# avik-pal/LocalRegNeuralDE.jl

Measured on NVIDIA B200. Metric: mnist_ode_train_samples_per_s, higher is better.
Workload: dtype tf32x3

## Files before the change

localregneuralde.jl_b200/csrc/lrnde_adjoint.cu:

```cuda
#include "lrnde_adjoint.h"

#include <stdio.h>
#include <stdlib.h>
#include <string.h>

#include <algorithm>

#include "lrnde_fused_dev.cuh"

enum {
  LA_ALPHA = 0,
  LA_S1 = 2,
  LA_DEL = 8,
  LA_CC = 13,
  LA_HH = 18,
  LA_EPS = 23,
  LA_DBT = 29,
  LA_HBB = 30,
  LA_HBT = 31,
  LA_NARR = 32
};

#ifdef LRNDE_UMMA_TRACE
__device__ long long g_adj_trace[1024];
// ... 158 lines not shown
        }
        bulk_commit();
        bulk_wait0();
      }
      __syncwarp();
    }
  } else if (warp == 1) {
    constexpr uint32_t idesc = make_idesc(128, kNT / 2);
    mbar_wait(&a_ready, 0);
    tc_fence_after();
    const uint32_t mz_hi = tmem_base, mz_lo = tmem_base + (uint32_t)(8 * p.KS);
    const uint32_t mt_hi = tmem_base + (uint32_t)(16 * p.KS), mt_lo = tmem_base + (uint32_t)(24 * p.KS);
    for (int st = 0; st < nst; ++st) {
      const uint32_t ph = (uint32_t)(st & 1);
      for (int cg = 0; cg < 2; ++cg) {
        mbar_wait(&bfull[cg], ph);
        tc_fence_after();
        if (elect_one_sync()) {
          if (cg == 0 && !SINGLE) ATRACE(7, st);
          issue_group(c_acc + (uint32_t)(cg * 32), mz_hi, mz_lo, smem_u32(tC[cg]), p.nfull, p.ntail, p.passes, idesc);
          mma_commit(&pdone[cg]);
          if (cg == 0 && !SINGLE) ATRACE(8, st);
        }
        __syncwarp();
      }
      if (!SINGLE) {
        for (int cg = 0; cg < 2; ++cg) {
          mbar_wait(&pread[cg], ph);
          tc_fence_after();
          if (elect_one_sync()) {
            issue_group(c_acc + (uint32_t)(cg * 32), mt_hi, mt_lo, smem_u32(tE[cg]), p.nfull, p.ntail, p.passes, idesc);
            mma_commit(&xdone[cg]);
          }
          __syncwarp();
        }
      }
    }
  } else {
    const int q = warp & 3, sub = (warp - 2) >> 2;
    const int cg = sub >> 1;
    const int hrow = q * 32 + lane;
    const uint32_t tlane = tmem_base + ((uint32_t)(q * 32) << 16);
    const int rbase = (sub & 1) * 16;
    const int nb = n0 + cg * 32 + rbase;
    const bool rowv = hrow < p.H;
    const bool rowc = hrow < p.Kaug;
    {
#pragma unroll
      for (int j = 0; j < 4; ++j) {
        const int ks = sub + 4 * j;
        if (ks < p.KS) {
          float a1[8], a2[8], hi[8], lo[8];
#pragma unroll
          for (int e = 0; e < 8; ++e) {
            const int k = ks * 8 + e;
            a1[e] = __ldg(p.Mz + hrow * 128 + k);
            a2[e] = (rowv && k < p.H) ? __ldg(p.Mz + k * 128 + hrow) : 0.0f;
          }
#pragma unroll
          for (int e = 0; e < 8; ++e) {
            if (p.passes == 3) { hi[e] = tf32_rna(a1[e]); lo[e] = tf32_rna(a1[e] - hi[e]); }
            else { hi[e] = a1[e]; lo[e] = 0.0f; }
          }
          tmem_st8(tlane + (uint32_t)(ks * 8), hi);
          tmem_st8(tlane + (uint32_t)(8 * p.KS + ks * 8), lo);
#pragma unroll
          for (int e = 0; e < 8; ++e) {
            if (p.passes == 3) { hi[e] = tf32_rna(a2[e]); lo[e] = tf32_rna(a2[e] - hi[e]); }
            else { hi[e] = a2[e]; lo[e] = 0.0f; }
          }
          tmem_st8(tlane + (uint32_t)(16 * p.KS + ks * 8), hi);
          tmem_st8(tlane + (uint32_t)(24 * p.KS + ks * 8), lo);
        }
      }
    }
    tmem_st_wait();
    tc_fence_before();
    __syncwarp();
    if (lane == 0) mbar_arrive(&a_ready);
    if (tr) ATRACE(0, 1);

    const bool in_full = hrow < p.nfull * 32;
    const bool in_img = hrow < p.KS * 8;
    uint32_t oA, oS, oLo, osw;
    if (in_full) {
      oS = 128u; oLo = 4096u; osw = (uint32_t)(lane >> 2);
      oA = (uint32_t)(q * 8192 + (lane & 3) * 4) + (uint32_t)rbase * oS;
    } else {
      const int kt = hrow - p.nfull * 32, t = kt >> 3, kk = kt & 7;
      oS = 32u; oLo = 1024u; osw = (uint32_t)((kk >> 2) & 1);
      oA = (uint32_t)(p.nfull * 8192 + t * 2048 + (kk & 3) * 4) + (uint32_t)rbase * oS;
    }
    const uint32_t rnd = (p.passes == 3) ? 0x1000u : 0u, msk = (p.passes == 3) ? 0xFFFFE000u : 0xFFFFFFFFu;
    auto tile_put16 = [&](uint8_t* tile, const float (&val)[16]) {
      if (!in_img) return;
#pragma unroll
      for (int i = 0; i < 16; ++i) {
        const uint32_t m = in_full ? (uint32_t)(i & 7) : (uint32_t)((i >> 2) & 1);
        const uint32_t o = oA + (uint32_t)i * oS + ((osw ^ m) << 4);
        const float hi = __uint_as_float((__float_as_uint(val[i]) + rnd) & msk);
        const float lo = __uint_as_float((__float_as_uint(val[i] - hi) + rnd) & msk);
        *reinterpret_cast<float*>(tile + o) = hi;
        *reinterpret_cast<float*>(tile + o + oLo) = lo;
      }
    };
    const float w1t = (p.td && rowv && p.w1t) ? p.w1t[hrow] : 0.0f;
    const float b1 = rowv ? p.b1[hrow] : 0.0f;
    const int slot = s_slot, next = s_next;
    const float dt = sd[0].scale;
    const float* alpha_n = SINGLE ? p.alpha_in : arr(LA_ALPHA + slot);
    const size_t e0 = (size_t)nb * LR_ZROW + hrow;
    uint8_t* const tCc = tC[cg];
    uint8_t* const tEc = tE[cg];
    const float* tape_row = reinterpret_cast<const float*>(tbuf) + (cg * 32 + rbase) * LR_ZROW + hrow;

    float c[16], ep[16], dprev[16];
#pragma unroll
    for (int i = 0; i < 16; ++i) { c[i] = 0.0f; ep[i] = 0.0f; dprev[i] = 0.0f; }
    if (!SINGLE && rowv) {
      const float* d1 = arr(LA_S1 + 3 * slot + 0) + e0;
#pragma unroll
      for (int i = 0; i < 16; ++i) dprev[i] = __ldcg(d1 + (size_t)i * LR_ZROW);
    }
    float v[16], ss[16];
    for (int jj = -1; jj < nst; ++jj) {
      const LinComb& yd = SINGLE ? sy[0] : sy[jj < 0 ? 1 : jj + 1];
      const float tau = yd.t;
      const bool last = (!SINGLE && jj == 5);
      float* dst_del = SINGLE ? arr(LA_S1 + 3 * slot + 0) : (last ? arr(LA_S1 + 3 * next + 0) : arr(LA_DEL + max(jj, 0)));
      float* dst_hh = SINGLE ? arr(LA_S1 + 3 * slot + 1) : (last ? arr(LA_S1 + 3 * next + 1) : arr(LA_HH + max(jj, 0)));
      float* dst_cc = SINGLE ? arr(LA_S1 + 3 * slot + 2) : (last ? arr(LA_S1 + 3 * next + 2) : arr(LA_CC + max(jj, 0)));
      if (jj >= 0) {
        if (tr) ATRACE(1, jj);
        const float cextra = (hrow == p.Kaug) ? tau : ((hrow == p.Kaug + 1) ? 1.0f : 0.0f);
#pragma unroll
        for (int i = 0; i < 16; ++i) dst_cc[e0 + (size_t)i * LR_ZROW] = rowc ? c[i] : cextra;
        tile_put16(tCc, c);
        if (!SINGLE) {
          const float cl = sd[jj].coef[jj];
          float* dst_eps = arr(LA_EPS + jj) + e0;
#pragma unroll
          for (int i = 0; i < 16; ++i) { v[i] = fmaf(cl, dprev[i], ep[i]); dst_eps[(size_t)i * LR_ZROW] = v[i]; }
          tile_put16(tEc, v);
        }
        tc_fence_before();
        fence_proxy_async();
        __syncwarp();
        if (lane == 0) mbar_arrive(&bfull[cg]);
        if (tr) ATRACE(2, jj);
      }
      if (jj + 1 < nst) {
        const LinComb& yn = SINGLE ? sy[0] : sy[jj + 2];
#pragma unroll
        for (int i = 0; i < 16; ++i) c[i] = 0.0f;
        for (int s = 0; s < 8; ++s) {
          const int it = (jj + 1) * 8 + s;
          const int b = it % kTapeBufs;
          mbar_wait(&tfull[b], (uint32_t)((it / kTapeBufs) & 1));
          if (rowc) {
            const float* tb = tape_row + (size_t)b * (kTapeBufBytes / 4);
            const float cf = (s < 7) ? yn.coef[s] : 1.0f, sc = (s < 7) ? 1.0f : yn.scale;
#pragma unroll
            for (int i = 0; i < 16; ++i) c[i] = fmaf(cf, tb[i * LR_ZROW], sc * c[i]);
          }
          __syncwarp();
          if (lane == 0) mbar_arrive(&tempty[b]);
        }
        if (!SINGLE && jj >= 0) {
#pragma unroll
          for (int i = 0; i < 16; ++i) ep[i] = sd[jj + 1].coef[jj] * dprev[i];
          if (rowv) {
            for (int s = 0; s < jj; ++s) {
              const float* src = ((s == 0) ? arr(LA_S1 + 3 * slot + 0) : arr(LA_DEL + s - 1)) + e0;
              const float cf = sd[jj + 1].coef[s];
#pragma unroll
              for (int i = 0; i < 16; ++i) ep[i] = fmaf(cf, __ldcg(src + (size_t)i * LR_ZROW), ep[i]);
            }
          }
        }
      }
      if (jj >= 0) {
        if (tr) ATRACE(3, jj);
#pragma unroll
        for (int i = 0; i < 16; ++i) ss[i] = rowv ? __ldcg(p.Zx + e0 + (size_t)i * LR_ZROW) : 0.0f;
        mbar_wait(&pdone[cg], (uint32_t)(jj & 1));
        if (tr) ATRACE(4, jj);
// ... 236 lines not shown
            if (pvec && row + 3 < o.prows) r = __ldcg(reinterpret_cast<const float4*>(pp));
            else {
              if (row + 0 < o.prows) r.x = __ldcg(pp + 0);
              if (row + 1 < o.prows) r.y = __ldcg(pp + 1);
              if (row + 2 < o.prows) r.z = __ldcg(pp + 2);
              if (row + 3 < o.prows) r.w = __ldcg(pp + 3);
            }
          } else if (g < 4) {
            r = __ldcg(reinterpret_cast<const float4*>(o.Q0 + (size_t)b * LR_ZROW + c4 * 4));
          } else if (o.Q1) {
            r = __ldcg(reinterpret_cast<const float4*>(o.Q1 + (size_t)b * LR_ZROW + c4 * 4));
          }
        }
        dst[g] = r;
      }
    };
    if (niter > 0) load_iter(0, v[0]);
    if (niter > 1) load_iter(1, v[1]);
    for (int it0 = 0; it0 < niter; it0 += 2) {
#pragma unroll
      for (int dd = 0; dd < 2; ++dd) {
        const int it = it0 + dd;
        if (it < niter) {
          const int s = it % NS, ph = (it / NS) & 1;
          uint8_t* stage = smem + (size_t)s * kPaStageBytes;
          const Ops o = ops_of(it);
          mbar_wait(&empty_bar[s], (uint32_t)(ph ^ 1));
#pragma unroll
          for (int g = 0; g < 6; ++g) {
            const int li = tid + (g & 1) * PT;
            const int bl = li >> 5, c4 = li & 31;
            const int grp = c4 >> 3, c32 = (c4 & 7) >> 1, half = c4 & 1, k4 = bl >> 2, r = bl & 3;
            const uint32_t off = (uint32_t)((k4 * 4 + grp) * 512 + r * 128 + ((c32 ^ r) << 5) + half * 16);
            float4 xv = (g >= 4 && !o.Q1) ? v[dd][g - 2] : v[dd][g];
            const float sc = (g < 2) ? 1.0f : ((g < 4) ? o.s0 : o.s1);
            xv.x *= sc; xv.y *= sc; xv.z *= sc; xv.w *= sc;
            float4 hi, lo;
            if (q.passes == 3) {
              hi = make_float4(tf32_rna(xv.x), tf32_rna(xv.y), tf32_rna(xv.z), tf32_rna(xv.w));
              lo = make_float4(tf32_rna(xv.x - hi.x), tf32_rna(xv.y - hi.y), tf32_rna(xv.z - hi.z), tf32_rna(xv.w - hi.w));
            } else { hi = xv; lo = make_float4(0.f, 0.f, 0.f, 0.f); }
            uint8_t* img = stage + (g >> 1) * 32768;
            *reinterpret_cast<float4*>(img + off) = hi;
            *reinterpret_cast<float4*>(img + 16384 + off) = lo;
          }
          if (it + 2 < niter) load_iter(it + 2, v[dd]);
          fence_proxy_async();
          __syncwarp();
          if (lane == 0) mbar_arrive(&full_bar[s]);
        }
      }
    }
    mbar_wait(&done_bar, 0);
    tc_fence_after();
    const int quarter = (warp & 3) * 32;
    const int wgroup = (warp - 2) >> 2;
    const int mrow = quarter + lane;
    const int nacc = (job == 0) ? 4 : 2;
    float* out;
    if (job == 0) out = q.partP + (size_t)split * 4 * 16384;
    else out = (job == 1 ? q.partX : q.partL) + ((size_t)split * q.ntile + tile) * 2 * 16384;
    for (int a = 0; a < nacc; ++a) {
      for (int cb = wgroup; cb < 8; cb += kEpiWarps / 4) {
        float r[16];
        tmem_ld16(tmem_base + ((uint32_t)quarter << 16) + (uint32_t)(a * 128 + cb * 16), r);
        float4* o4 = reinterpret_cast<float4*>(out + (size_t)a * 16384 + (size_t)mrow * 128 + cb * 16);
        if (niter == 0) {
#pragma unroll
          for (int j = 0; j < 16; ++j) r[j] = 0.0f;
        }
#pragma unroll
        for (int j = 0; j < 4; ++j) o4[j] = make_float4(r[4 * j], r[4 * j + 1], r[4 * j + 2], r[4 * j + 3]);
      }
    }
    tc_fence_before();
  }
  __syncthreads();
  if (warp == 1) {
    tc_fence_after();
    asm volatile("tcgen05.dealloc.cta_group::1.sync.aligned.b32 %0, %1;" ::"r"(tmem_base), "r"(512u) : "memory");
  }
}

struct AReduceP {
  SolveDev* S;
  const float* partP; const float* partX; const float* partL;
  float* RP; float* RX; float* RL;
  int nP, nD, ntile;
};
__global__ void __launch_bounds__(256) adj_reduce_kernel(AReduceP p) {
  if (p.S->done) return;
  const size_t nP4 = 4 * 4096, nX4 = (size_t)p.ntile * 2 * 4096;
  for (size_t i = blockIdx.x * (size_t)blockDim.x + threadIdx.x; i < nP4 + 2 * nX4; i += (size_t)gridDim.x * blockDim.x) {
    float4 s = make_float4(0.f, 0.f, 0.f, 0.f);
    if (i < nP4) {
      const float4* src = reinterpret_cast<const float4*>(p.partP) + i;
#pragma unroll 8
      for (int k = 0; k < p.nP; ++k) {
        const float4 v = __ldcg(src + (size_t)k * nP4);
        s.x += v.x; s.y += v.y; s.z += v.z; s.w += v.w;
      }
      reinterpret_cast<float4*>(p.RP)[i] = s;
    } else {
      const bool isx = (i - nP4) < nX4;
      const size_t j = isx ? (i - nP4) : (i - nP4 - nX4);
      const float4* src = reinterpret_cast<const float4*>(isx ? p.partX : p.partL) + j;
      for (int k = 0; k < p.nD; ++k) {
        const float4 v = __ldcg(src + (size_t)k * nX4);
        s.x += v.x; s.y += v.y; s.z += v.z; s.w += v.w;
      }
      const size_t tile = j / (2 * 4096), rem = j % (2 * 4096), vv = rem / 4096, mn = rem % 4096;
      float4* dst = reinterpret_cast<float4*>(isx ? p.RX : p.RL);
      dst[(vv * p.ntile + tile) * 4096 + mn] = s;
    }
  }
}

struct AMuP {
  SolveDev* S;
  const float* RP; const float* RX; const float* RL;
  const float* W2a;
  const float* W1T;
  int D, H, td, Kaug, ntile;
  long w1_off, w2_off;
  long nparams;
};
__global__ void __launch_bounds__(512) adj_mu_kernel(AMuP p) {
  SolveDev* S = p.S;
  if (S->done) return;
  const int slot = S->slot, next = (S->slot + 1) % S->cap;
  const float* mu_n = lr_slot_u(S, slot) + S->lam_len;
  float* mu_new = lr_slot_u(S, next) + S->lam_len;
  const float dt = S->err.scale, abstol = S->abstol, reltol = S->reltol;
  const int H = p.H, D = p.D, Kaug = p.Kaug;
  const long n1 = (long)H * (D + p.td + 1), n2 = (long)D * Kaug;
  const size_t RXs = (size_t)p.ntile * 128 * 128;
  const bool multi = S->reduce_mu && S->nranks > 1;
  const int par = (int)(S->mseq & 1ull);
  float* st0 = multi ? lr_mbox_stage(S->mbox[S->rank], par, 0) : nullptr;
  float* st1 = multi ? lr_mbox_stage(S->mbox[S->rank], par, 1) : nullptr;
  double acc = 0.0;
  for (long i = blockIdx.x * (long)blockDim.x + threadIdx.x; i < n1 + n2; i += (long)gridDim.x * blockDim.x) {
    float g0, g1;
    long pidx;
    if (i < n1) {
      const int d = (int)(i / H), r = (int)(i % H);
      pidx = p.w1_off + i;
      if (d < D) {
        float a0 = p.RX[(size_t)d * 128 + r], a1 = p.RX[RXs + (size_t)d * 128 + r];
        const float* w = p.W2a + d;
        const float* P0 = p.RP + r;
        const float* P1 = p.RP + 16384 + r;
#pragma unroll 8
        for (int k = 0; k < Kaug; ++k) {
          const float wv = __ldg(w + (size_t)k * D);
          a0 = fmaf(P0[k * 128], wv, a0);
          a1 = fmaf(P1[k * 128], wv, a1);
        }
        g0 = a0; g1 = a1;
      } else {
        const int krow = (p.td && d == D) ? Kaug : Kaug + 1;
        g0 = p.RP[(size_t)krow * 128 + r];
        g1 = p.RP[16384 + (size_t)krow * 128 + r];
      }
    } else {
      const long i2 = i - n1;
      const int k = (int)(i2 / D), d = (int)(i2 % D);
      pidx = p.w2_off + i2;
      float a0 = 0.0f, a1 = 0.0f;
      const float* P0 = p.RP + 2 * 16384 + (size_t)k * 128;
      const float* P1 = p.RP + 3 * 16384 + (size_t)k * 128;
      const float* w = p.W1T + d;
#pragma unroll 8
      for (int r = 0; r < H; ++r) {
        const float wv = __ldg(w + (size_t)r * D);
        a0 = fmaf(P0[r], wv, a0);
        a1 = fmaf(P1[r], wv, a1);
      }
      g0 = fmaf(-dt, a0, p.RL[(size_t)d * 128 + k]);
      g1 = fmaf(-dt, a1, p.RL[RXs + (size_t)d * 128 + k]);
    }
    if (multi) {
      st0[pidx] = g0;
      st1[pidx] = g1;
      continue;
    }
    const float mn = mu_n[pidx];
    const float mv = fmaf(-dt, g0, mn);
    mu_new[pidx] = mv;
    const float ut = -dt * g1;
    const float r = ut / (abstol + fmaxf(fabsf(mn), fabsf(mv)) * reltol);
    acc += (double)(r * r);
  }
  if (multi) {
    __threadfence_system();
    __syncthreads();
    if (threadIdx.x == 0) {
      const unsigned int prev = atomicAdd(S->mucounter, 1u);
      if (prev == gridDim.x - 1) {
        *S->mucounter = 0;
        __threadfence_system();
        for (int r = 0; r < S->nranks; ++r) {
          volatile unsigned long long* f = &S->mbox[r]->mflag[par][S->rank];
          *f = S->mseq + 1;
        }
      }
    }
    return;
  }
  __shared__ double sh[16];
  for (int o = 16; o > 0; o >>= 1) acc += __shfl_down_sync(0xffffffffu, acc, o);
  if ((threadIdx.x & 31) == 0) sh[threadIdx.x >> 5] = acc;
  __syncthreads();
  if (threadIdx.x == 0) {
    double s = 0.0;
    for (int w = 0; w < (int)(blockDim.x >> 5); ++w) s += sh[w];
    S->partials[LR_ERR_BLOCKS + blockIdx.x] = s;
  }
}

__global__ void __launch_bounds__(256) adj_mu_finish_kernel(SolveDev* S) {
  if (S->done) return;
  const int par = (int)(S->mseq & 1ull);
  LrMailbox* mine = S->mbox[S->rank];
  if (threadIdx.x == 0) {
    long long spins = 0;
    for (int r = 0; r < S->nranks; ++r) {
      volatile unsigned long long* f = &mine->mflag[par][r];
      while (*f != S->mseq + 1) {
        __nanosleep(40);
        if (++spins > (1ll << 26)) { lr_peer_timeout(S); break; }
      }
    }
    __threadfence_system();
  }
  __syncthreads();
  const int slot = S->slot, next = (S->slot + 1) % S->cap;
  const size_t P = S->mu_len;
  const float* mu_n = lr_slot_u(S, slot) + S->lam_len;
  float* mu_new = lr_slot_u(S, next) + S->lam_len;
  const float* mg_n = S->muglob + (size_t)slot * P;
  float* mg_new = S->muglob + (size_t)next * P;
  const float* own0 = lr_mbox_stage(mine, par, 0);
  const float dt = S->err.scale, abstol = S->abstol, reltol = S->reltol;
  double acc = 0.0;
  for (size_t i = blockIdx.x * (size_t)blockDim.x + threadIdx.x; i < P; i += (size_t)gridDim.x * blockDim.x) {
    float g0 = 0.0f, g1 = 0.0f;
    for (int r = 0; r < S->nranks; ++r) {
      g0 += ((const volatile float*)lr_mbox_stage(S->mbox[r], par, 0))[i];
      g1 += ((const volatile float*)lr_mbox_stage(S->mbox[r], par, 1))[i];
    }
    mu_new[i] = fmaf(-dt, ((const volatile float*)own0)[i], mu_n[i]);
    const float mn = mg_n[i];
    const float mv = fmaf(-dt, g0, mn);
    mg_new[i] = mv;
    const float ut = -dt * g1;
    const float rr = ut / (abstol + fmaxf(fabsf(mn), fabsf(mv)) * reltol);
    acc += (double)(rr * rr);
  }
  __shared__ double sh[8];
  for (int o = 16; o > 0; o >>= 1) acc += __shfl_down_sync(0xffffffffu, acc, o);
  if ((threadIdx.x & 31) == 0) sh[threadIdx.x >> 5] = acc;
  __syncthreads();
  if (threadIdx.x == 0) {
    double s = 0.0;
    for (int w = 0; w < 8; ++w) s += sh[w];
    S->partials[LR_ERR_BLOCKS + blockIdx.x] = s;
  }
}

}

#define LRA_COUNT(ctx) do { if ((ctx)->capturing) (ctx)->captured++; else (ctx)->launches++; } while (0)

bool LatentAdjoint::eligible(const lrnde_model* m) {
  FusedShape s;
  if (!lrf_shape(m, &s)) return false;
  return s.KS <= 14 && s.Kaug + 2 <= 128;
}

LatentAdjoint::LatentAdjoint(lrnde_ctx* c, const lrnde_model* mm, const float* p, int64_t b, int npasses)
    : ctx(c), m(mm), ps(p), B(b), passes(npasses) {
  lrf_shape(m, &sh);
  ntiles = (int)((B + fused::kNT - 1) / fused::kNT);
  zlen = (size_t)LR_ZROW * (size_t)ntiles * fused::kNT;
  nunits = (int)((B + 15) / 16);
  unit_bytes = (size_t)sh.nfull * 8192 + (size_t)sh.ntail * 2048;
  const int maxc = std::max(1, 148 / sh.n_mt);
  const int rounds = (nunits + maxc - 1) / maxc;
  nclusters = (nunits + rounds - 1) / rounds;
  ntile_d = (sh.D + 127) / 128;
  const int nchunk_tot = (int)((B + 31) / 32);
  const double wP = 13.0, wD = 2.0 * ntile_d;
  int wantP = std::max(1, (int)(148.0 * wP / (wP + wD)));
  int cP = std::max(1, (nchunk_tot + wantP - 1) / wantP);
  chunkP = cP * 32;
  nP = (int)((B + chunkP - 1) / chunkP);
  int wantD = std::max(1, (148 - nP) / (2 * ntile_d));
  int cD = std::max(1, (nchunk_tot + wantD - 1) / wantD);
  chunkD = cD * 32;
  nD = (int)((B + chunkD - 1) / chunkD);
  Mz = (float*)ctx->alloc(sizeof(float) * 128 * 128);
  ws = (float*)ctx->alloc(sizeof(float) * LA_NARR * zlen);
  alpha_in = (float*)ctx->alloc(sizeof(float) * zlen);
  hbuf = (float*)ctx->alloc((size_t)ntiles * 4 * unit_bytes);
  partP = (float*)ctx->alloc(sizeof(float) * (size_t)nP * 4 * 16384);
  partX = (float*)ctx->alloc(sizeof(float) * (size_t)nD * ntile_d * 2 * 16384);
  partL = (float*)ctx->alloc(sizeof(float) * (size_t)nD * ntile_d * 2 * 16384);
  RP = (float*)ctx->alloc(sizeof(float) * 4 * 16384);
  RX = (float*)ctx->alloc(sizeof(float) * (size_t)ntile_d * 2 * 16384);
  RL = (float*)ctx->alloc(sizeof(float) * (size_t)ntile_d * 2 * 16384);
  static bool attr_set = false;
  if (!attr_set) {
    constexpr int kChainSmem = 4 * (3 * 8192 + 3 * 2048) + ladj::kTapeBufs * ladj::kTapeBufBytes + 1024;
    LR_CUDA(cudaFuncSetAttribute(ladj::adj_chain_kernel<ACT_IDENTITY, false>, cudaFuncAttributeMaxDynamicSharedMemorySize, kChainSmem));
    LR_CUDA(cudaFuncSetAttribute(ladj::adj_chain_kernel<ACT_IDENTITY, true>, cudaFuncAttributeMaxDynamicSharedMemorySize, kChainSmem));
    LR_CUDA(cudaFuncSetAttribute(ladj::adj_chain_kernel<ACT_TANH, false>, cudaFuncAttributeMaxDynamicSharedMemorySize, kChainSmem));
    LR_CUDA(cudaFuncSetAttribute(ladj::adj_chain_kernel<ACT_TANH, true>, cudaFuncAttributeMaxDynamicSharedMemorySize, kChainSmem));
    LR_CUDA(cudaFuncSetAttribute(ladj::adj_chain_kernel<ACT_GELU, false>, cudaFuncAttributeMaxDynamicSharedMemorySize, kChainSmem));
    LR_CUDA(cudaFuncSetAttribute(ladj::adj_chain_kernel<ACT_GELU, true>, cudaFuncAttributeMaxDynamicSharedMemorySize, kChainSmem));
    LR_CUDA(cudaFuncSetAttribute(ladj::adj_chain_kernel<ACT_SIGMOID, false>, cudaFuncAttributeMaxDynamicSharedMemorySize, kChainSmem));
    LR_CUDA(cudaFuncSetAttribute(ladj::adj_chain_kernel<ACT_SIGMOID, true>, cudaFuncAttributeMaxDynamicSharedMemorySize, kChainSmem));
    LR_CUDA(cudaFuncSetAttribute(ladj::adj_chain_kernel<ACT_RELU, false>, cudaFuncAttributeMaxDynamicSharedMemorySize, kChainSmem));
    LR_CUDA(cudaFuncSetAttribute(ladj::adj_chain_kernel<ACT_RELU, true>, cudaFuncAttributeMaxDynamicSharedMemorySize, kChainSmem));
    LR_CUDA(cudaFuncSetAttribute(ladj::pairacc_kernel, cudaFuncAttributeMaxDynamicSharedMemorySize, ladj::pairacc_smem()));
    attr_set = true;
  }
  if (getenv("LRNDE_FUSED_VERBOSE"))
    fprintf(stderr, "[lrnde adjoint] B=%lld tiles=%d units=%d kgemm clusters=%d pairacc: nP=%d x %d samples, nD=%d x %d samples x %d tiles\n",
            (long long)B, ntiles, nunits, nclusters, nP, chunkP, nD, chunkD, ntile_d);
}

LatentAdjoint::~LatentAdjoint() {
  ctx->release(Mz); ctx->release(ws); ctx->release(alpha_in); ctx->release(hbuf);
  ctx->release(partP); ctx->release(partX); ctx->release(partL);
  ctx->release(RP); ctx->release(RX); ctx->release(RL);
}

void LatentAdjoint::prepare(const float* mz_plain) {
  if (mz_plain) { Mz_ext = mz_plain; return; }
  lrf_mz_plain(ctx, m, ps, Mz);
  LRA_COUNT(ctx);
}

static void lra_launch_chain(LatentAdjoint& E, SolveDev* S, int single) {
  const FusedShape& sh = E.sh;
  const LayerInfo& L1 = E.m->layers[0];
  ladj::AChainP cp;
  memset(&cp, 0, sizeof(cp));
  cp.S = S; cp.single = single; cp.Mz = E.Mz_ext ? E.Mz_ext : E.Mz;
  cp.w1t = sh.td ? E.ps + L1.w_off + (size_t)sh.D * sh.H : nullptr;
  cp.b1 = E.ps + L1.b_off;
  cp.Zx = E.Zx; cp.alpha_in = E.alpha_in; cp.ws = E.ws; cp.zlen = E.zlen;
  cp.hbuf = E.hbuf; cp.unit_bytes = (uint32_t)E.unit_bytes;
  cp.B = (int)E.B; cp.H = sh.H; cp.td = sh.td; cp.Kaug = sh.Kaug; cp.KS = sh.KS; cp.nfull = sh.nfull; cp.ntail = sh.ntail;
  cp.passes = E.passes;
  const size_t smem_c = 4 * ((size_t)sh.nfull * 8192 + (size_t)sh.ntail * 2048) + ladj::kTapeBufs * ladj::kTapeBufBytes + 1024;
  cudaStream_t st = E.ctx->stream;
#define LRA_CHAIN(A) do { if (single) ladj::adj_chain_kernel<A, true><<<E.ntiles, fused::kThreads, smem_c, st>>>(cp); \
                         else ladj::adj_chain_kernel<A, false><<<E.ntiles, fused::kThreads, smem_c, st>>>(cp); } while (0)
  switch (sh.act) {
    case ACT_TANH: LRA_CHAIN(ACT_TANH); break;
    case ACT_GELU: LRA_CHAIN(ACT_GELU); break;
    case ACT_SIGMOID: LRA_CHAIN(ACT_SIGMOID); break;
    case ACT_RELU: LRA_CHAIN(ACT_RELU); break;
    default: LRA_CHAIN(ACT_IDENTITY); break;
  }
#undef LRA_CHAIN
  LRA_COUNT(E.ctx);
  LR_CUDA(cudaGetLastError());
}

static void lra_launch_pairacc(LatentAdjoint& E, SolveDev* S) {
  ladj::PairAccP q;
  memset(&q, 0, sizeof(q));
  q.S = S; q.ws = E.ws; q.zlen = E.zlen; q.x = E.x; q.D = E.sh.D; q.B = (int)E.B;
  q.nP = E.nP; q.chunkP = E.chunkP; q.nD = E.nD; q.chunkD = E.chunkD; q.ntile = E.ntile_d;
  q.partP = E.partP; q.partX = E.partX; q.partL = E.partL; q.passes = E.passes;
  int n = 0;
  for (int j = 1; j <= 7; ++j) {
    const float bj = (j <= 6) ? lr_tsit5_a(5, j - 1) : 0.0f;
    const float btj = lr_tsit5_btilde(j - 1);
    const int del = (j == 1) ? -1 : ((j == 7) ? -10 : LA_DEL + j - 2);
    const int hh = (j == 1) ? -2 : ((j == 7) ? -11 : LA_HH + j - 2);
    const int cc = (j == 1) ? -3 : ((j == 7) ? -12 : LA_CC + j - 2);
    q.term[n++] = {cc, del, bj, btj, 0};
    if (j >= 2) q.term[n++] = {hh, LA_EPS + j - 2, bj, btj, 1};
  }
  q.nterm = n;
  const int grid = E.nP + 2 * E.ntile_d * E.nD;
  ladj::pairacc_kernel<<<grid, fused::kThreads, ladj::pairacc_smem(), E.ctx->stream>>>(q);
  LRA_COUNT(E.ctx);
  LR_CUDA(cudaGetLastError());
}

static void lra_launch_mu(LatentAdjoint& E, SolveDev* S) {
  cudaStream_t st = E.ctx->stream;
  ladj::AReduceP r;
  r.S = S; r.partP = E.partP; r.partX = E.partX; r.partL = E.partL; r.RP = E.RP; r.RX = E.RX; r.RL = E.RL;
  r.nP = E.nP; r.nD = E.nD; r.ntile = E.ntile_d;
  const size_t n4 = 4 * 4096 + 2 * (size_t)E.ntile_d * 2 * 4096;
  ladj::adj_reduce_kernel<<<(int)((n4 + 255) / 256), 256, 0, st>>>(r);
  LRA_COUNT(E.ctx);
  const LayerInfo& L1 = E.m->layers[0];
  const LayerInfo& L2 = E.m->layers[1];
  ladj::AMuP mp;
  memset(&mp, 0, sizeof(mp));
  mp.S = S; mp.RP = E.RP; mp.RX = E.RX; mp.RL = E.RL;
  mp.W2a = E.ps + L2.w_off; mp.W1T = E.W1T;
  mp.D = E.sh.D; mp.H = E.sh.H; mp.td = E.sh.td; mp.Kaug = E.sh.Kaug; mp.ntile = E.ntile_d;
  mp.w1_off = (long)L1.w_off; mp.w2_off = (long)L2.w_off; mp.nparams = (long)E.m->nparams;
  ladj::adj_mu_kernel<<<LR_ERR_BLOCKS, 512, 0, st>>>(mp);
  LRA_COUNT(E.ctx);
  if (E.ctx->nranks > 1) {
    ladj::adj_mu_finish_kernel<<<LR_ERR_BLOCKS, 256, 0, st>>>(S);
    LRA_COUNT(E.ctx);
  }
  LR_CUDA(cudaGetLastError());
}

void LatentAdjoint::begin(SolveDev* S) { lra_launch_chain(*this, S, 1); }

void LatentAdjoint::attempt(SolveDev* S) {
  lra_launch_chain(*this, S, 0);
  lrf_launch_kgemm_adj(ctx, S, sh, ps + m->layers[0].w_off, hbuf, unit_bytes, B, passes, nunits, nclusters);
  lra_launch_pairacc(*this, S);
  lra_launch_mu(*this, S);
}

void LatentAdjoint::attempt_part(SolveDev* S, int which) {
  if (which == 0) lra_launch_chain(*this, S, 0);
  else if (which == 1) lrf_launch_kgemm_adj(ctx, S, sh, ps + m->layers[0].w_off, hbuf, unit_bytes, B, passes, nunits, nclusters);
  else if (which == 2) lra_launch_pairacc(*this, S);
  else lra_launch_mu(*this, S);
}
```

localregneuralde.jl_b200/csrc/lrnde_adjoint.h:

```cpp
#pragma once
#include "lrnde_fused.h"

struct LatentAdjoint {
  lrnde_ctx* ctx;
  const lrnde_model* m;
  const float* ps;
  int64_t B;
  int passes;
  FusedShape sh;
  size_t zlen = 0;
  int ntiles = 0, nunits = 0, nclusters = 1;
  int ntile_d = 0;
  int nP = 1, chunkP = 32;
  int nD = 1, chunkD = 32;
  float* Mz = nullptr;
  const float* Mz_ext = nullptr;
  float* ws = nullptr;
  float* alpha_in = nullptr;
  float* hbuf = nullptr;
  size_t unit_bytes = 0;
  float* partP = nullptr; float* partX = nullptr; float* partL = nullptr;
  float* RP = nullptr; float* RX = nullptr; float* RL = nullptr;
  const float* W1T = nullptr;
  const float* Zx = nullptr;
  const float* x = nullptr;

  static bool eligible(const lrnde_model* m);
  LatentAdjoint(lrnde_ctx* c, const lrnde_model* mm, const float* p, int64_t b, int npasses);
  ~LatentAdjoint();
  void prepare(const float* mz_plain = nullptr);
  void begin(SolveDev* S);
  void attempt(SolveDev* S);
  void attempt_part(SolveDev* S, int which);
};
```

Baseline: 1.086 million.

## Fuse partial-block reduction into adjoint mu kernel and simplify tile operand stores

Removes the separate adj_reduce_kernel and its RP/RX/RL buffers. The mu kernel now sums the per-chunk partials directly: hidden-space partials are reduced into shared memory per 4-row block, and the x/lambda partials are reduced per column in registers. Each thread then handles 4 parameter rows with float4 FMAs, which cuts one launch and one round trip through global memory but repeats some partial reads across blocks. The chain kernel's tile_put16 is also split into separate full and tail address paths that read laneid directly, so less offset state is precomputed. Unused partials slots are zeroed because the grid can now be smaller than LR_ERR_BLOCKS.

```diff
diff --git a/localregneuralde.jl_b200/csrc/lrnde_adjoint.cu b/localregneuralde.jl_b200/csrc/lrnde_adjoint.cu
--- a/localregneuralde.jl_b200/csrc/lrnde_adjoint.cu
+++ b/localregneuralde.jl_b200/csrc/lrnde_adjoint.cu
@@ -264,26 +264,37 @@
 
     const bool in_full = hrow < p.nfull * 32;
     const bool in_img = hrow < p.KS * 8;
-    uint32_t oA, oS, oLo, osw;
-    if (in_full) {
-      oS = 128u; oLo = 4096u; osw = (uint32_t)(lane >> 2);
-      oA = (uint32_t)(q * 8192 + (lane & 3) * 4) + (uint32_t)rbase * oS;
-    } else {
-      const int kt = hrow - p.nfull * 32, t = kt >> 3, kk = kt & 7;
-      oS = 32u; oLo = 1024u; osw = (uint32_t)((kk >> 2) & 1);
-      oA = (uint32_t)(p.nfull * 8192 + t * 2048 + (kk & 3) * 4) + (uint32_t)rbase * oS;
-    }
     const uint32_t rnd = (p.passes == 3) ? 0x1000u : 0u, msk = (p.passes == 3) ? 0xFFFFE000u : 0xFFFFFFFFu;
     auto tile_put16 = [&](uint8_t* tile, const float (&val)[16]) {
       if (!in_img) return;
-#pragma unroll
-      for (int i = 0; i < 16; ++i) {
-        const uint32_t m = in_full ? (uint32_t)(i & 7) : (uint32_t)((i >> 2) & 1);
-        const uint32_t o = oA + (uint32_t)i * oS + ((osw ^ m) << 4);
-        const float hi = __uint_as_float((__float_as_uint(val[i]) + rnd) & msk);
-        const float lo = __uint_as_float((__float_as_uint(val[i] - hi) + rnd) & msk);
-        *reinterpret_cast<float*>(tile + o) = hi;
-        *reinterpret_cast<float*>(tile + o + oLo) = lo;
+      uint32_t ln;
+      asm volatile("mov.u32 %0, %%laneid;" : "=r"(ln));
+      auto split = [&](float x) {
+        const float hi = __uint_as_float((__float_as_uint(x) + rnd) & msk);
+        const float lo = __uint_as_float((__float_as_uint(x - hi) + rnd) & msk);
+        return make_float2(hi, lo);
+      };
+      if (in_full) {
+        uint8_t* base = tile + q * 8192 + (ln & 3) * 4 + rbase * 128;
+        const uint32_t xr = (ln >> 2) << 4;
+#pragma unroll
+        for (int i = 0; i < 16; ++i) {
+          uint8_t* at = base + i * 128 + (xr ^ (uint32_t)((i & 7) << 4));
+          const float2 h = split(val[i]);
+          *reinterpret_cast<float*>(at) = h.x;
+          *reinterpret_cast<float*>(at + 4096) = h.y;
+        }
+      } else {
+        const int kt = q * 32 + (int)ln - p.nfull * 32, t = kt >> 3, kk = kt & 7;
+        uint8_t* base = tile + p.nfull * 8192 + t * 2048 + (kk & 3) * 4 + rbase * 32;
+        const uint32_t xr = (uint32_t)((kk >> 2) & 1) << 4;
+#pragma unroll
+        for (int i = 0; i < 16; ++i) {
+          uint8_t* at = base + i * 32 + (xr ^ (uint32_t)(((i >> 2) & 1) << 4));
+          const float2 h = split(val[i]);
+          *reinterpret_cast<float*>(at) = h.x;
+          *reinterpret_cast<float*>(at + 1024) = h.y;
+        }
       }
     };
     const float w1t = (p.td && rowv && p.w1t) ? p.w1t[hrow] : 0.0f;
@@ -686,115 +697,128 @@
   }
 }
 
-struct AReduceP {
+constexpr int kMuRows = 4, kMuThreads = 256;
+struct AMuP {
   SolveDev* S;
   const float* partP; const float* partX; const float* partL;
-  float* RP; float* RX; float* RL;
   int nP, nD, ntile;
-};
-__global__ void __launch_bounds__(256) adj_reduce_kernel(AReduceP p) {
-  if (p.S->done) return;
-  const size_t nP4 = 4 * 4096, nX4 = (size_t)p.ntile * 2 * 4096;
-  for (size_t i = blockIdx.x * (size_t)blockDim.x + threadIdx.x; i < nP4 + 2 * nX4; i += (size_t)gridDim.x * blockDim.x) {
-    float4 s = make_float4(0.f, 0.f, 0.f, 0.f);
-    if (i < nP4) {
-      const float4* src = reinterpret_cast<const float4*>(p.partP) + i;
-#pragma unroll 8
-      for (int k = 0; k < p.nP; ++k) {
-        const float4 v = __ldcg(src + (size_t)k * nP4);
-        s.x += v.x; s.y += v.y; s.z += v.z; s.w += v.w;
-      }
-      reinterpret_cast<float4*>(p.RP)[i] = s;
-    } else {
-      const bool isx = (i - nP4) < nX4;
-      const size_t j = isx ? (i - nP4) : (i - nP4 - nX4);
-      const float4* src = reinterpret_cast<const float4*>(isx ? p.partX : p.partL) + j;
-      for (int k = 0; k < p.nD; ++k) {
-        const float4 v = __ldcg(src + (size_t)k * nX4);
-        s.x += v.x; s.y += v.y; s.z += v.z; s.w += v.w;
-      }
-      const size_t tile = j / (2 * 4096), rem = j % (2 * 4096), vv = rem / 4096, mn = rem % 4096;
-      float4* dst = reinterpret_cast<float4*>(isx ? p.RX : p.RL);
-      dst[(vv * p.ntile + tile) * 4096 + mn] = s;
-    }
-  }
-}
-
-struct AMuP {
-  SolveDev* S;
-  const float* RP; const float* RX; const float* RL;
   const float* W2a;
   const float* W1T;
-  int D, H, td, Kaug, ntile;
+  int D, H, td, Kaug;
+  int cpt;
+  int nb1, ncb1, ncb2;
   long w1_off, w2_off;
-  long nparams;
 };
-__global__ void __launch_bounds__(512) adj_mu_kernel(AMuP p) {
+__global__ void __launch_bounds__(kMuThreads, 1) adj_mu_kernel(AMuP p) {
   SolveDev* S = p.S;
   if (S->done) return;
+  __shared__ __align__(16) float sR[2 * 128 * kMuRows];
   const int slot = S->slot, next = (S->slot + 1) % S->cap;
   const float* mu_n = lr_slot_u(S, slot) + S->lam_len;
   float* mu_new = lr_slot_u(S, next) + S->lam_len;
   const float dt = S->err.scale, abstol = S->abstol, reltol = S->reltol;
   const int H = p.H, D = p.D, Kaug = p.Kaug;
-  const long n1 = (long)H * (D + p.td + 1), n2 = (long)D * Kaug;
-  const size_t RXs = (size_t)p.ntile * 128 * 128;
+  const bool w1 = (int)blockIdx.x < p.nb1 * p.ncb1;
+  const int b = w1 ? (int)blockIdx.x : (int)blockIdx.x - p.nb1 * p.ncb1;
+  const int ncb = w1 ? p.ncb1 : p.ncb2;
+  const int row0 = (b / ncb) * kMuRows, col0 = (b % ncb) * p.cpt * kMuThreads;
+  const int tid = threadIdx.x;
+  constexpr size_t kBlk = 16384;
+
+  {
+    const int nitem = w1 ? 2 * (Kaug + 2) : 2 * kMuRows * 32;
+    for (int it = tid; it < nitem; it += kMuThreads) {
+      size_t off;
+      int w, k = 0, kk = 0, f = 0;
+      if (w1) { w = it / (Kaug + 2); k = it % (Kaug + 2); off = (size_t)w * kBlk + (size_t)k * 128 + row0; }
+      else { w = it / (kMuRows * 32); kk = (it / 32) % kMuRows; f = it % 32; off = (size_t)(2 + w) * kBlk + (size_t)(row0 + kk) * 128 + 4 * f; }
+      const float4* src = reinterpret_cast<const float4*>(p.partP + off);
+      float4 s = make_float4(0.f, 0.f, 0.f, 0.f);
+#pragma unroll 8
+      for (int sp = 0; sp < p.nP; ++sp) {
+        const float4 v = __ldcg(src + (size_t)sp * (4 * kBlk / 4));
+        s.x += v.x; s.y += v.y; s.z += v.z; s.w += v.w;
+      }
+      if (w1) *reinterpret_cast<float4*>(sR + (w * 128 + k) * kMuRows) = s;
+      else {
+        float* dst = sR + (w * 128 + 4 * f) * kMuRows + kk;
+        dst[0] = s.x; dst[kMuRows] = s.y; dst[2 * kMuRows] = s.z; dst[3 * kMuRows] = s.w;
+      }
+    }
+  }
+  __syncthreads();
+
   const bool multi = S->reduce_mu && S->nranks > 1;
   const int par = (int)(S->mseq & 1ull);
   float* st0 = multi ? lr_mbox_stage(S->mbox[S->rank], par, 0) : nullptr;
   float* st1 = multi ? lr_mbox_stage(S->mbox[S->rank], par, 1) : nullptr;
+  const int ncols = w1 ? D + p.td + 1 : D;
+  const int nrows = min(kMuRows, (w1 ? H : Kaug) - row0);
+  const size_t dstride = (size_t)p.ntile * 2 * kBlk;
   double acc = 0.0;
-  for (long i = blockIdx.x * (long)blockDim.x + threadIdx.x; i < n1 + n2; i += (long)gridDim.x * blockDim.x) {
-    float g0, g1;
-    long pidx;
-    if (i < n1) {
-      const int d = (int)(i / H), r = (int)(i % H);
-      pidx = p.w1_off + i;
-      if (d < D) {
-        float a0 = p.RX[(size_t)d * 128 + r], a1 = p.RX[RXs + (size_t)d * 128 + r];
+#pragma unroll 1
+  for (int cc = 0; cc < p.cpt; ++cc) {
+    const int d = col0 + cc * kMuThreads + tid;
+    if (d >= ncols) break;
+    static_assert(kMuRows == 4, "one float4 of rows per column");
+    float4 g0, g1;
+    if (d < D) {
+      const float4* src = reinterpret_cast<const float4*>((w1 ? p.partX : p.partL) + (size_t)(d >> 7) * 2 * kBlk +
+                                                          (size_t)(d & 127) * 128 + row0);
+      float4 e0 = make_float4(0.f, 0.f, 0.f, 0.f), e1 = e0;
+      for (int sp = 0; sp < p.nD; ++sp) {
+        const float4 v0 = __ldcg(src + (size_t)sp * (dstride / 4)), v1 = __ldcg(src + (size_t)sp * (dstride / 4) + kBlk / 4);
+        e0.x += v0.x; e0.y += v0.y; e0.z += v0.z; e0.w += v0.w;
+        e1.x += v1.x; e1.y += v1.y; e1.z += v1.z; e1.w += v1.w;
+      }
+      const float4* R0 = reinterpret_cast<const float4*>(sR);
+      const float4* R1 = reinterpret_cast<const float4*>(sR + 128 * kMuRows);
+      if (w1) {
+        float4 a0 = e0, a1 = e1;
         const float* w = p.W2a + d;
-        const float* P0 = p.RP + r;
-        const float* P1 = p.RP + 16384 + r;
 #pragma unroll 8
         for (int k = 0; k < Kaug; ++k) {
           const float wv = __ldg(w + (size_t)k * D);
-          a0 = fmaf(P0[k * 128], wv, a0);
-          a1 = fmaf(P1[k * 128], wv, a1);
+          const float4 q0 = R0[k], q1 = R1[k];
+          a0.x = fmaf(q0.x, wv, a0.x); a0.y = fmaf(q0.y, wv, a0.y); a0.z = fmaf(q0.z, wv, a0.z); a0.w = fmaf(q0.w, wv, a0.w);
+          a1.x = fmaf(q1.x, wv, a1.x); a1.y = fmaf(q1.y, wv, a1.y); a1.z = fmaf(q1.z, wv, a1.z); a1.w = fmaf(q1.w, wv, a1.w);
         }
         g0 = a0; g1 = a1;
       } else {
-        const int krow = (p.td && d == D) ? Kaug : Kaug + 1;
-        g0 = p.RP[(size_t)krow * 128 + r];
-        g1 = p.RP[16384 + (size_t)krow * 128 + r];
+        float4 a0 = make_float4(0.f, 0.f, 0.f, 0.f), a1 = a0;
+        const float* w = p.W1T + d;
+#pragma unroll 8
+        for (int r = 0; r < H; ++r) {
+          const float wv = __ldg(w + (size_t)r * D);
+          const float4 q0 = R0[r], q1 = R1[r];
+          a0.x = fmaf(q0.x, wv, a0.x); a0.y = fmaf(q0.y, wv, a0.y); a0.z = fmaf(q0.z, wv, a0.z); a0.w = fmaf(q0.w, wv, a0.w);
+          a1.x = fmaf(q1.x, wv, a1.x); a1.y = fmaf(q1.y, wv, a1.y); a1.z = fmaf(q1.z, wv, a1.z); a1.w = fmaf(q1.w, wv, a1.w);
+        }
+        g0 = make_float4(fmaf(-dt, a0.x, e0.x), fmaf(-dt, a0.y, e0.y), fmaf(-dt, a0.z, e0.z), fmaf(-dt, a0.w, e0.w));
+        g1 = make_float4(fmaf(-dt, a1.x, e1.x), fmaf(-dt, a1.y, e1.y), fmaf(-dt, a1.z, e1.z), fmaf(-dt, a1.w, e1.w));
       }
     } else {
-      const long i2 = i - n1;
-      const int k = (int)(i2 / D), d = (int)(i2 % D);
-      pidx = p.w2_off + i2;
-      float a0 = 0.0f, a1 = 0.0f;
-      const float* P0 = p.RP + 2 * 16384 + (size_t)k * 128;
-      const float* P1 = p.RP + 3 * 16384 + (size_t)k * 128;
-      const float* w = p.W1T + d;
-#pragma unroll 8
-      for (int r = 0; r < H; ++r) {
-        const float wv = __ldg(w + (size_t)r * D);
-        a0 = fmaf(P0[r], wv, a0);
-        a1 = fmaf(P1[r], wv, a1);
-      }
-      g0 = fmaf(-dt, a0, p.RL[(size_t)d * 128 + k]);
-      g1 = fmaf(-dt, a1, p.RL[RXs + (size_t)d * 128 + k]);
-    }
-    if (multi) {
-      st0[pidx] = g0;
-      st1[pidx] = g1;
-      continue;
-    }
-    const float mn = mu_n[pidx];
-    const float mv = fmaf(-dt, g0, mn);
-    mu_new[pidx] = mv;
-    const float ut = -dt * g1;
-    const float r = ut / (abstol + fmaxf(fabsf(mn), fabsf(mv)) * reltol);
-    acc += (double)(r * r);
+      const int krow = (p.td && d == D) ? Kaug : Kaug + 1;
+      g0 = reinterpret_cast<const float4*>(sR)[krow];
+      g1 = reinterpret_cast<const float4*>(sR)[128 + krow];
+    }
+    const float o0[kMuRows] = {g0.x, g0.y, g0.z, g0.w}, o1[kMuRows] = {g1.x, g1.y, g1.z, g1.w};
+#pragma unroll
+    for (int e = 0; e < kMuRows; ++e) {
+      if (e >= nrows) continue;
+      const long pidx = w1 ? p.w1_off + (long)d * H + row0 + e : p.w2_off + (long)(row0 + e) * D + d;
+      if (multi) {
+        st0[pidx] = o0[e];
+        st1[pidx] = o1[e];
+        continue;
+      }
+      const float mn = mu_n[pidx];
+      const float mv = fmaf(-dt, o0[e], mn);
+      mu_new[pidx] = mv;
+      const float ut = -dt * o1[e];
+      const float r = ut / (abstol + fmaxf(fabsf(mn), fabsf(mv)) * reltol);
+      acc += (double)(r * r);
+    }
   }
   if (multi) {
     __threadfence_system();
@@ -820,6 +844,7 @@
     double s = 0.0;
     for (int w = 0; w < (int)(blockDim.x >> 5); ++w) s += sh[w];
     S->partials[LR_ERR_BLOCKS + blockIdx.x] = s;
+    for (int i = blockIdx.x + gridDim.x; i < LR_ERR_BLOCKS; i += gridDim.x) S->partials[LR_ERR_BLOCKS + i] = 0.0;
   }
 }
 
@@ -911,9 +936,6 @@
   partP = (float*)ctx->alloc(sizeof(float) * (size_t)nP * 4 * 16384);
   partX = (float*)ctx->alloc(sizeof(float) * (size_t)nD * ntile_d * 2 * 16384);
   partL = (float*)ctx->alloc(sizeof(float) * (size_t)nD * ntile_d * 2 * 16384);
-  RP = (float*)ctx->alloc(sizeof(float) * 4 * 16384);
-  RX = (float*)ctx->alloc(sizeof(float) * (size_t)ntile_d * 2 * 16384);
-  RL = (float*)ctx->alloc(sizeof(float) * (size_t)ntile_d * 2 * 16384);
   static bool attr_set = false;
   if (!attr_set) {
     constexpr int kChainSmem = 4 * (3 * 8192 + 3 * 2048) + ladj::kTapeBufs * ladj::kTapeBufBytes + 1024;
@@ -938,7 +960,6 @@
 LatentAdjoint::~LatentAdjoint() {
   ctx->release(Mz); ctx->release(ws); ctx->release(alpha_in); ctx->release(hbuf);
   ctx->release(partP); ctx->release(partX); ctx->release(partL);
-  ctx->release(RP); ctx->release(RX); ctx->release(RL);
 }
 
 void LatentAdjoint::prepare(const float* mz_plain) {
@@ -1000,21 +1021,26 @@
 
 static void lra_launch_mu(LatentAdjoint& E, SolveDev* S) {
   cudaStream_t st = E.ctx->stream;
-  ladj::AReduceP r;
-  r.S = S; r.partP = E.partP; r.partX = E.partX; r.partL = E.partL; r.RP = E.RP; r.RX = E.RX; r.RL = E.RL;
-  r.nP = E.nP; r.nD = E.nD; r.ntile = E.ntile_d;
-  const size_t n4 = 4 * 4096 + 2 * (size_t)E.ntile_d * 2 * 4096;
-  ladj::adj_reduce_kernel<<<(int)((n4 + 255) / 256), 256, 0, st>>>(r);
-  LRA_COUNT(E.ctx);
   const LayerInfo& L1 = E.m->layers[0];
   const LayerInfo& L2 = E.m->layers[1];
   ladj::AMuP mp;
   memset(&mp, 0, sizeof(mp));
-  mp.S = S; mp.RP = E.RP; mp.RX = E.RX; mp.RL = E.RL;
+  mp.S = S; mp.partP = E.partP; mp.partX = E.partX; mp.partL = E.partL;
+  mp.nP = E.nP; mp.nD = E.nD; mp.ntile = E.ntile_d;
   mp.W2a = E.ps + L2.w_off; mp.W1T = E.W1T;
-  mp.D = E.sh.D; mp.H = E.sh.H; mp.td = E.sh.td; mp.Kaug = E.sh.Kaug; mp.ntile = E.ntile_d;
-  mp.w1_off = (long)L1.w_off; mp.w2_off = (long)L2.w_off; mp.nparams = (long)E.m->nparams;
-  ladj::adj_mu_kernel<<<LR_ERR_BLOCKS, 512, 0, st>>>(mp);
+  mp.D = E.sh.D; mp.H = E.sh.H; mp.td = E.sh.td; mp.Kaug = E.sh.Kaug;
+  mp.w1_off = (long)L1.w_off; mp.w2_off = (long)L2.w_off;
+  constexpr int R = ladj::kMuRows;
+  int grid = 0;
+  for (mp.cpt = 2;; ++mp.cpt) {
+    const int C = mp.cpt * ladj::kMuThreads;
+    mp.nb1 = (E.sh.H + R - 1) / R;
+    mp.ncb1 = (E.sh.D + E.sh.td + 1 + C - 1) / C;
+    mp.ncb2 = (E.sh.D + C - 1) / C;
+    grid = mp.nb1 * mp.ncb1 + ((E.sh.Kaug + R - 1) / R) * mp.ncb2;
+    if (grid <= LR_ERR_BLOCKS) break;
+  }
+  ladj::adj_mu_kernel<<<grid, ladj::kMuThreads, 0, st>>>(mp);
   LRA_COUNT(E.ctx);
   if (E.ctx->nranks > 1) {
     ladj::adj_mu_finish_kernel<<<LR_ERR_BLOCKS, 256, 0, st>>>(S);
diff --git a/localregneuralde.jl_b200/csrc/lrnde_adjoint.h b/localregneuralde.jl_b200/csrc/lrnde_adjoint.h
--- a/localregneuralde.jl_b200/csrc/lrnde_adjoint.h
+++ b/localregneuralde.jl_b200/csrc/lrnde_adjoint.h
@@ -20,7 +20,6 @@
   float* hbuf = nullptr;
   size_t unit_bytes = 0;
   float* partP = nullptr; float* partX = nullptr; float* partL = nullptr;
-  float* RP = nullptr; float* RX = nullptr; float* RL = nullptr;
   const float* W1T = nullptr;
   const float* Zx = nullptr;
   const float* x = nullptr;
diff --git a/scratch/adj_traffic.py b/scratch/adj_traffic.py
--- /dev/null
+++ b/scratch/adj_traffic.py
@@ -0,0 +1,90 @@
+import argparse
+import json
+
+
+def shapes(B, D, H, td=1):
+    Kaug = H + td + 1
+    ntiles = (B + 63) // 64
+    KS = (Kaug + 2 + 7) // 8
+    nfull, ntail = KS // 4, KS % 4
+    unit_bytes = nfull * 8192 + ntail * 2048
+    ntile_d = (D + 127) // 128
+    nchunk_tot = (B + 31) // 32
+    wP, wD = 13.0, 2.0 * ntile_d
+    wantP = max(1, int(148.0 * wP / (wP + wD)))
+    cP = max(1, (nchunk_tot + wantP - 1) // wantP)
+    chunkP = cP * 32
+    nP = (B + chunkP - 1) // chunkP
+    wantD = max(1, (148 - nP) // (2 * ntile_d))
+    cD = max(1, (nchunk_tot + wantD - 1) // wantD)
+    chunkD = cD * 32
+    nD = (B + chunkD - 1) // chunkD
+    return dict(B=B, D=D, H=H, td=td, Kaug=Kaug, ntiles=ntiles, unit_bytes=unit_bytes, ntile_d=ntile_d, nP=nP, nD=nD)
+
+
+def count(s):
+    B, D, H, Kaug = s["B"], s["D"], s["H"], s["Kaug"]
+    Z = s["ntiles"] * 64 * 128 * 4
+    XD = D * B * 4
+    blk = 128 * 128 * 4
+    hbuf = s["ntiles"] * 4 * s["unit_bytes"]
+    P = H * (D + s["td"] + 1) + D * Kaug
+    W = (H * D + D * Kaug) * 4
+    chain = {
+        "tape: 6 stages x 8 tiles": 48 * Z,
+        "delta_1 + partial eps (10 earlier deltas)": 11 * Z,
+        "Zx and alpha_n, reloaded per stage": 12 * Z,
+        "closing gather (6 deltas, 7 [h;tau;1])": 13 * Z,
+        "stores: c, [h;tau;1], delta, eps per stage": 24 * Z,
+        "stores: alpha_{n+1}, Delta_bt, HB_b, HB_bt": 4 * Z,
+        "stores: Delta_b / Delta_bt operand images": hbuf,
+    }
+    kgemm = {"operand images": hbuf, "lambda_n": XD, "lambda_{n+1}": XD}
+    part_p = s["nP"] * 4 * blk
+    part_xl = 2 * s["nD"] * s["ntile_d"] * 2 * blk
+    pairacc = {
+        "hidden-space terms: 13 x (P, Q)": 26 * Z,
+        "x and lambda_n": 2 * XD,
+        "Delta_b, Delta_bt, HB_b, HB_bt per 128-feature tile": 2 * s["ntile_d"] * 2 * Z,
+        "partial blocks out": part_p + part_xl,
+    }
+    reduced = 4 * blk + 2 * s["ntile_d"] * 2 * blk
+    old_reduce = {"partial blocks in": part_p + part_xl, "RP / RX / RL out": reduced}
+    old_mu = {"RP / RX / RL in": reduced, "W2a, W1^T": W, "mu_n in, mu_{n+1} out": 2 * P * 4}
+    cols = 2 * 256
+    ncb1, ncb2 = (D + s["td"] + 1 + cols - 1) // cols, (D + cols - 1) // cols
+    nb1, nb2 = (H + 3) // 4, (Kaug + 3) // 4
+    new_mu = {
+        "hidden-space partials (slice per block)": s["nP"] * 4 * (nb1 * ncb1 * 2 * (Kaug + 2) * 4 + nb2 * ncb2 * 2 * 4 * 128),
+        "x / lambda_n partials": part_xl,
+        "W2a, W1^T (per row block)": 4 * (nb1 * D * Kaug + nb2 * H * D),
+        "mu_n in, mu_{n+1} out": 2 * P * 4,
+    }
+    old = {"adj_chain_kernel": chain, "kgemm_kernel<2,1>": kgemm, "pairacc_kernel": pairacc,
+           "adj_reduce_kernel": old_reduce, "adj_mu_kernel": old_mu}
+    new = {"adj_chain_kernel": chain, "kgemm_kernel<2,1>": kgemm, "pairacc_kernel": pairacc, "adj_mu_kernel (fused)": new_mu}
+    return old, new
+
+
+def main():
+    ap = argparse.ArgumentParser()
+    ap.add_argument("--batch", type=int, default=8192)
+    ap.add_argument("--D", type=int, default=784)
+    ap.add_argument("--H", type=int, default=100)
+    a = ap.parse_args()
+    s = shapes(a.batch, a.D, a.H)
+    old, new = count(s)
+    out = {"shape": s}
+    for tag, launches in (("old", old), ("new", new)):
+        tot = 0
+        rows = {}
+        for k, parts in launches.items():
+            b = sum(parts.values())
+            tot += b
+            rows[k] = {"MB": round(b / 1e6, 1), "parts_MB": {n: round(v / 1e6, 2) for n, v in parts.items()}}
+        out[tag] = {"launches": len(launches), "total_MB": round(tot / 1e6, 1), "per_launch": rows}
+    print(json.dumps(out, indent=1))
+
+
+if __name__ == "__main__":
+    main()
```

New measurement: 1.181 million (median of 6 runs). 1.09x the previous value.
